# indianajohn/akaze-rust

Hardware: AMD Instinct MI355X
Metric: Mpix/s through extract_features (4 oct x 4 sub) (higher is better)
Workload: dtype f32

## Files before the change

akaze-rust_amd/csrc/akz_api.cpp:

```cpp
#include <cstdio>

#include "akz_ctx.hpp"

unsigned akz::host_cpu_share() {
    unsigned n = std::max(1u, std::thread::hardware_concurrency());
    cpu_set_t set;
    if (sched_getaffinity(0, sizeof(set), &set) == 0) n = std::max(1, CPU_COUNT(&set));
    if (FILE* f = fopen("/sys/fs/cgroup/cpu.max", "r")) {
        char q[32] = {0};
        long period = 0;
        if (fscanf(f, "%31s %ld", q, &period) == 2 && period > 0 && strcmp(q, "max") != 0)
            n = std::min<unsigned>(n, (unsigned)std::max(1L, atol(q) / period));
        fclose(f);
    }
    if (const char* e = std::getenv("LOCAL_WORLD_SIZE")) {
        const int ranks = atoi(e);
        if (ranks > 1) n = std::max(2u, n / (unsigned)ranks);
    }
    return std::max(1u, n);
}

int level_info_out(const std::vector<LevelPlan>& plan, uint64_t level, double* etime, double* esigma,
                          uint32_t* octave, uint32_t* sublevel, uint32_t* sigma_size, uint32_t* lw, uint32_t* lh,
                          uint32_t* det_sigma, uint64_t* n_tau, double* tau, uint64_t tau_cap) {
// ... 295 lines not shown
}
int akz_ctx_set_match_mode(akz_ctx* c, int mode) {
    AKZ_TRY(bind(c));
    if (mode < 0 || mode > 3) return AKZ_ERR_INVALID_ARG;
    c->settings.match_mode = mode;
    push_settings(c);
    return AKZ_OK;
}
int akz_ctx_set_fed_mode(akz_ctx* c, int mode) {
    AKZ_TRY(bind(c));
    if (mode != 0 && mode != 2) return AKZ_ERR_INVALID_ARG;
    c->settings.fed_mode = mode;
    push_settings(c);
    return AKZ_OK;
}
const char* akz_fed_kernel_name(void) { return "k_level_march + k_fed_own"; }
int akz_debug_march_bands(int kind, uint32_t w, uint32_t h, uint32_t n, int half_width, int32_t* rows, uint32_t cap,
                          uint32_t* n_bands) {
    if (!n_bands || (cap && !rows) || kind < 0 || kind > 1 || w < 16 || h < 16 || n == 0 || half_width < 1 || half_width > 4)
        return AKZ_ERR_INVALID_ARG;
    *n_bands = launch::march_band_rows(kind, w, h, n, half_width, rows, cap);
    return AKZ_OK;
}
int akz_debug_detector_set_cells(int half_width, const uint32_t* w, const uint32_t* h, uint32_t n_entries, uint32_t n, int32_t* cells,
                                 uint32_t cap, int32_t* grids, uint32_t* n_workgroups) {
    if (!n_workgroups || !w || !h || !grids || (cap && !cells) || n_entries < 1 || n_entries > launch::detector_march_set_max() || n == 0 ||
        half_width < 1 || half_width > 4)
        return AKZ_ERR_INVALID_ARG;
    for (uint32_t e = 0; e < n_entries; ++e)
        if (w[e] < 4u * (uint32_t)half_width + 8u || h[e] < 4u * (uint32_t)half_width + 8u) return AKZ_ERR_INVALID_ARG;
    *n_workgroups = launch::detector_set_cells(half_width, w, h, n_entries, n, cells, cap, grids);
    return AKZ_OK;
}
const char* akz_detector_kernel_name(void) { return "detector (k_detector_march + k_detector_tiled)"; }
int akz_debug_set_schedule(akz_ctx* c, int key, int value) {
    if (!c || key < 0 || key >= SCHED_COUNT_) return AKZ_ERR_INVALID_ARG;
    AKZ_TRY(bind(c));
    CtxSettings& s = c->settings;
    s.sched[key] = value;
    if (key == SCHED_DET_BAND_ROWS || key == SCHED_LEVEL_BAND_ROWS)
        launch::march_min_band_rows(s.sched[SCHED_DET_BAND_ROWS], s.sched[SCHED_LEVEL_BAND_ROWS]);
    if (key == SCHED_DET_SETS) launch::detector_set_waves(value >= 11 && value <= 14 ? value - 10 : 0);
    if (key == SCHED_JOB_KPX) {
        s.big_px_sync = value > 0 ? (uint64_t)value * 1000u : gates::kBigPxSync;
        s.big_px_async = value > 0 ? (uint64_t)value * 1000u : gates::kBigPxAsync;
        s.lane_px = value > 0 ? (uint64_t)value * 1000u : gates::kLanePx;
    }
    push_settings(c);
    return AKZ_OK;
}
int akz_debug_placement_verdict(float spin_pair_ms, float tiny_pair_ms, float tiny_alone_ms, float spin_ms) {
    return akz::placement_verdict(spin_pair_ms, tiny_pair_ms, tiny_alone_ms, spin_ms);
}
int akz_debug_stream_placement(akz_ctx* c, int* info) {
    if (!c || !info) return AKZ_ERR_INVALID_ARG;
    AKZ_TRY(bind(c));
    info[0] = c->placed ? 1 : 0;
    info[1] = c->pre_mode;
    info[2] = c->place_replaced;
    info[3] = c->place_collisions + c->lane_collisions;
    return AKZ_OK;
}
int akz_debug_select_info(akz_ctx* c, int* info) {
    if (!c || !info) return AKZ_ERR_INVALID_ARG;
    AKZ_TRY(bind(c));
    const akz_ctx* q = c->lanes.empty() ? c : c->lanes[0];
    info[0] = q->sel_last_mode.load();
    info[1] = (int)q->sel_last_rounds.load();
    info[2] = (int)q->sel_last_fallback.load();
    info[3] = (int)q->last_total_cands.load();
    for (int k = 0; k < 4; ++k) info[4 + k] = (int)q->sel_last_ticks[k].load();
    return AKZ_OK;
}
int akz_debug_set_select(akz_ctx* c, int mode) {
    if (!c) return AKZ_ERR_INVALID_ARG;
// ... 140 lines not shown
```

akaze-rust_amd/csrc/akz_internal.hpp:

```cpp
#pragma once
#include <hip/hip_runtime.h>

#include <cstdint>
#include <functional>
#include <string>
#include <vector>

#include "../../include/akaze_hip.h"
#include "../../include/akaze_hip_debug.h"

namespace akz {

void set_error(const std::string& msg);
unsigned host_cpu_share();

using TrialsOnDevice = std::function<int(const float*, const float*, const float*, const float*, uint32_t, const uint32_t*, uint32_t,
                                         float, float, float*, int32_t*)>;
int remove_outliers_impl(const akz_keypoint* keypoints_0, uint64_t n0, const akz_keypoint* keypoints_1, uint64_t n1,
                         const akz_match* matches, uint64_t n_matches, uint64_t num_trials, float epsilon_model,
                         float epsilon_inlier, akz_match* out, uint64_t* n_out, const TrialsOnDevice& trials_on_device);

#define AKZ_HIP_TRY(expr)                                                                          \
    do {                                                                                           \
        hipError_t _e = (expr);                                                                    \
// ... 156 lines not shown
    uint32_t w, h, level;
    float border_m;
};
uint32_t detector_tiled_set_max();
void detector_tiled_set(hipStream_t s, uint32_t sigma, const DetLevelDesc* levels, uint32_t nlevels, uint32_t n, float thr,
                        Candidate* d_cand, uint32_t cap, uint32_t* d_count);
void detector_tiled_fused(hipStream_t s, const float* lsmooth, uint32_t sigma, float* lx, float* ly, float* lxx,
                          float* lyy, float* lxy, float* ldet_out, uint32_t w, uint32_t h, uint32_t n, uint32_t level,
                          float thr, float border_m, Candidate* d_cand, uint32_t cap, uint32_t* d_count);
bool blur5_stream_supported(uint32_t w, uint32_t h, uint32_t ntaps, bool is_u8);
void blur5_stream_u8(hipStream_t s, const uint8_t* in, float* out, uint32_t w, uint32_t h, uint32_t n, const float* k);
void blur5_stream_f32(hipStream_t s, const float* in, float* out, uint32_t w, uint32_t h, uint32_t n, const float* k);
uint32_t march_band_rows(int kind, uint32_t w, uint32_t h, uint32_t n, int S, int32_t* cs_ce, uint32_t cap);
bool blur5_march_supported(uint32_t w, uint32_t h, uint32_t ntaps);
void blur5_march_u8(hipStream_t s, const uint8_t* in, float* out, uint32_t w, uint32_t h, uint32_t n, const float* k);
void blur5_march_f32(hipStream_t s, const float* in, float* out, uint32_t w, uint32_t h, uint32_t n, const float* k);
bool contrast_march_supported(uint32_t w, uint32_t h, uint32_t ntaps, uint32_t nbins);
void contrast_march(hipStream_t s, const float* in, uint32_t w, uint32_t h, uint32_t n, const float* g3,
                    unsigned long long* d_hmax_bits, uint32_t nbins, uint32_t* d_hist, double* d_thr);
void contrast_thresholds(hipStream_t s, const unsigned long long* d_hmax_bits, uint32_t nbins, uint32_t n, double* d_thr);
bool contrast_stream_supported(uint32_t w, uint32_t h, uint32_t ntaps, uint32_t nbins);
void contrast_stream(hipStream_t s, const float* in, uint32_t w, uint32_t h, uint32_t n, const float* g3,
                     unsigned long long* d_hmax_bits, uint32_t nbins, uint32_t* d_hist, double* d_thr);
bool prep_stream_supported(uint32_t w, uint32_t h);
void prep_stream(hipStream_t s, const float* prev, bool half, float* lt_out, float* lsmooth, float* lflow, uint32_t w,
                 uint32_t h, uint32_t pw, uint32_t ph, uint32_t n, const float* g3, const double* d_k, uint32_t k_pow);
bool detector_march_supported(uint32_t sigma, uint32_t w, uint32_t h, float border_m, bool nms);
void detector_march(hipStream_t s, const float* lsmooth, uint32_t sigma, float* lx, float* ly, float* lxx, float* lyy,
                    float* lxy, float* ldet_out, uint32_t w, uint32_t h, uint32_t n, uint32_t level, float thr,
                    float border_m, Candidate* d_cand, uint32_t cap, uint32_t* d_count);
uint32_t detector_march_set_max();
void detector_march_set(hipStream_t s, uint32_t sigma, const DetLevelDesc* levels, uint32_t nlevels, uint32_t n, float thr,
                        Candidate* d_cand, uint32_t cap, uint32_t* d_count);
void detector_set_waves(int waves);
uint32_t detector_set_cells(int S, const uint32_t* w, const uint32_t* h, uint32_t nlv, uint32_t n, int32_t* cells, uint32_t cap,
                            int32_t* grids);
bool head_fused_supported(uint32_t w, uint32_t h, uint32_t ntaps0, uint32_t ntaps1);
void head_fused_u8(hipStream_t s, const uint8_t* in, float* lt0, float* blurred, float* gx, float* gy, uint32_t w, uint32_t h, uint32_t n,
                   const float* k5, const float* g3, unsigned long long* d_smax_bits, uint32_t* d_zero_word = nullptr);
void head_fused_f32(hipStream_t s, const float* in, float* lt0, float* blurred, float* gx, float* gy, uint32_t w, uint32_t h, uint32_t n,
                    const float* k5, const float* g3, unsigned long long* d_smax_bits, uint32_t* d_zero_word = nullptr);
void contrast_hist_final(hipStream_t s, const float* gx, const float* gy, uint32_t w, uint32_t h, uint32_t n, unsigned long long* d_smax_bits,
                         uint32_t nbins, uint32_t* d_hist, uint32_t* d_done, double percentile, double* d_k);
void flow_from_pair(hipStream_t s, const float* gx, const float* gy, float* lflow, uint32_t w, uint32_t h, uint32_t n, const double* d_k,
                    uint32_t k_pow);
void march_min_band_rows(int detector, int level);
bool level_march_supported(uint32_t w, uint32_t h);
bool level_march_half_supported(uint32_t w, uint32_t h, uint32_t pw, uint32_t ph, uint32_t n_steps);
void level_march(hipStream_t s, const float* prev, float* lsmooth, float* lflow, float* lt_out, float* lstep, uint32_t w,
                 uint32_t h, uint32_t n, const float* g3, const double* d_k, uint32_t k_pow, const float* half_taus,
                 uint32_t n_steps, uint32_t pw = 0, uint32_t ph = 0);
struct ResidentLevel {
    float *lt, *lsmooth, *lflow, *lstep;
    uint32_t w, h;
    bool half;
    uint32_t n_tau;
    const float* half_tau;
    uint32_t k_pow;
};
constexpr int kResidentMaxLevels = 10;
constexpr int kResidentMaxSteps = 448;
bool octave_resident_supported(uint32_t w, uint32_t h);
void octave_resident(hipStream_t s, const float* prev, uint32_t pw, uint32_t ph, uint32_t n, const ResidentLevel* levels,
                     uint32_t n_levels, const float* g3, const double* d_k);
bool detector_nms_fused_supported(uint32_t sigma);
void detector_nms_fused(hipStream_t s, const float* lsmooth, uint32_t sigma, float* lx, float* ly, float* lxx,
                        float* lyy, float* lxy, float* ldet_out, uint32_t w, uint32_t h, uint32_t n, uint32_t level,
                        float thr, float border_m, Candidate* d_cand, uint32_t cap, uint32_t* d_count);
void rcp_f64_to_f32(hipStream_t s, const double* x, float* out, uint64_t n);
// ... 172 lines not shown
```

akaze-rust_amd/csrc/akz_march.hip:

```cpp
#include <hip/hip_runtime.h>

#include <algorithm>
#include <cstdlib>
#include <type_traits>

#include "akz_internal.hpp"
#include "akz_pm_g2.hpp"

namespace akz {
namespace {

typedef float f2 __attribute__((ext_vector_type(2)));
typedef float f2u __attribute__((ext_vector_type(2), aligned(4)));

constexpr int MT = 256;
constexpr int MW = 2 * MT;
constexpr int HALO = 16;
constexpr int USE = MW - 2 * HALO;
constexpr int PAD = 8;
constexpr int ROW = MW + 2 * PAD;
constexpr int CBUF = 32;
#ifndef AKZ_MARCH_PF
#define AKZ_MARCH_PF 3
#endif
// ... 11 lines not shown
    return (int)((blockIdx.x & 7u) * (gridDim.x >> 3) + (blockIdx.x >> 3));
#else
    return (int)blockIdx.x;
#endif
}
__host__ __device__ __forceinline__ void uniform_band_rows(const MarchGrid& g, int band, int S, int h, int* cs, int* ce) {
    *cs = S + band * g.band_rows;
    const int e = *cs + g.band_rows;
    *ce = e < h - S ? e : h - S;
}
__host__ __device__ __forceinline__ void level_band_rows(const MarchGrid& g, int band, int h, int* cs, int* ce) {
    *cs = 1 + (band == 0 ? 0 : g.edge_rows + (band - 1) * g.band_rows);
    const int e = *cs + (band == 0 ? g.edge_rows : g.band_rows);
    *ce = band == g.nbands - 1 ? h - 1 : (e < h - 1 ? e : h - 1);
}
struct MarchNms {
    unsigned level;
    float thr;
    int xlo, xhi, ylo, yhi;
    Candidate* cand;
    unsigned cap;
    unsigned* count;
};

constexpr int kDetSetMax = 4;
struct DetMarchEntry {
    const float* ls;
    float *lx, *ly, *ldet, *lxx, *lyy, *lxy;
    int w, h;
    MarchGrid g;
    unsigned level;
    int xlo, xhi, ylo, yhi;
    int first;
};
struct DetMarchSet {
    DetMarchEntry e[kDetSetMax];
};
#if defined(__HIP_DEVICE_COMPILE__)
#define AKZ_UNIFORM(x) __builtin_amdgcn_readfirstlane(x)
#else
#define AKZ_UNIFORM(x) (x)
#endif
__host__ __device__ __forceinline__ bool det_set_cell(const DetMarchSet& set, int wg, int nwg, DetMarchEntry* E, int* entry, int* img,
                                                      int* band, int* strip) {
#if AKZ_MARCH_XCD
    const int xcd = wg & 7, j = wg >> 3;
    (void)nwg;
#else
    const int xcd = wg / (nwg >> 3), j = wg - xcd * (nwg >> 3);
#endif
    DetMarchEntry X = set.e[0];
    int e = 0, jl = j;
    const int f1 = set.e[1].first, f2 = set.e[2].first, f3 = set.e[3].first;
    if (j >= f1) { X = set.e[1]; e = 1; jl = j - f1; }
    if (j >= f2) { X = set.e[2]; e = 2; jl = j - f2; }
    if (j >= f3) { X = set.e[3]; e = 3; jl = j - f3; }
    static_assert(kDetSetMax == 4, "compare chain");
    const int cell = AKZ_UNIFORM(xcd * ((X.g.total + 7) >> 3) + jl);
    if (cell >= X.g.total) return false;
    const int per = X.g.nbands * X.g.nstrips;
    const int i = AKZ_UNIFORM(cell / per);
    const int rem = cell - i * per;
    const int b = AKZ_UNIFORM(rem / X.g.nstrips);
    *E = X;
    *entry = e;
    *img = i;
    *band = b;
    *strip = rem - b * X.g.nstrips;
    return true;
}

__device__ __forceinline__ int clampi(int v, int lo, int hi) { return v < lo ? lo : (v > hi ? hi : v); }
__device__ __forceinline__ f2 tap_main(f2 a, f2 b, f2 c, float kn, float kwn) {
    const f2 z = {0.0f, 0.0f};
    return ((z + kn * a) + kwn * b) + kn * c;
}
__device__ __forceinline__ f2 tap_off(f2 a, f2 c) {
    const f2 z = {0.0f, 0.0f};
    return (z - a) + c;
}

__device__ __forceinline__ void cands_flush(Candidate* buf, unsigned& n, const MarchNms& nms, int lane) {
    if (n == 0) return;
    unsigned base = 0;
    if (lane == 0) base = atomicAdd(nms.count, n);
    base = (unsigned)__builtin_amdgcn_readfirstlane((int)base);
    const uint4* src = reinterpret_cast<const uint4*>(buf);
    uint4* dst = reinterpret_cast<uint4*>(nms.cand);
    for (unsigned e = (unsigned)lane; e < 2u * n; e += 64u)
        if (base + (e >> 1) < nms.cap) dst[2 * (size_t)base + e] = src[e];
    __builtin_amdgcn_wave_barrier();
    n = 0;
}
template <typename F>
__device__ __forceinline__ void cands_push(Candidate* buf, unsigned& n, unsigned m, const MarchNms& nms, int lane, F&& make) {
    while (__ballot(m != 0u)) {
        const bool have = m != 0u;
        const int i = have ? __ffs(m) - 1 : 0;
        m &= m - 1u;
        const unsigned long long b = __ballot(have);
        const unsigned nb = (unsigned)__popcll(b);
        if (n + nb > (unsigned)CBUF) cands_flush(buf, n, nms, lane);
        const unsigned before = (unsigned)__popcll(b & ((1ull << lane) - 1ull));
// ... 68 lines not shown
    constexpr int AUX = NT ? 2 : 0;
    if (!ODDW) {
        const unsigned vo = on ? C.vo_st : VO_NONE;
#pragma unroll
        for (int i = 0; i < N; ++i)
            __builtin_amdgcn_raw_buffer_store_b64(__builtin_bit_cast(u2, v[i]), plane[i], (int)vo, (int)ro, AUX);
    } else {
        const unsigned vo0 = on ? C.vo_st : VO_NONE, vo1 = on ? C.vo_st1 : VO_NONE;
#pragma unroll
        for (int i = 0; i < N; ++i) {
            const float a = v[i].x, b = v[i].y;
            __builtin_amdgcn_raw_buffer_store_b32(__float_as_uint(a), plane[i], (int)vo0, (int)ro, AUX);
            __builtin_amdgcn_raw_buffer_store_b32(__float_as_uint(b), plane[i], (int)vo1, (int)ro, AUX);
        }
    }
}
template <int S, int N, bool ODDW, bool NT = true>
__device__ __forceinline__ void store_filled(const __amdgpu_buffer_rsrc_t (&plane)[N], const Cols& C, int w, int h, int r, bool on,
                                             const f2 (&v)[N]) {
    store_rows<N, ODDW, NT>(plane, r, w, on, C, v);
    if (on && (r == S || r == h - 1 - S)) {
        if (r == S) {
#pragma nounroll
            for (int y = 0; y < S; ++y) store_rows<N, ODDW, NT>(plane, y, w, true, C, v);
        }
        if (r == h - 1 - S) {
#pragma nounroll
            for (int y = h - S; y < h; ++y) store_rows<N, ODDW, NT>(plane, y, w, true, C, v);
        }
    }
}

template <int S, bool NMS, bool KEEP, bool ODDW>
__global__ void __launch_bounds__(MT, 3)
k_detector_march(DetMarchSet set, float kn, float kwn, float quat, float thr, Candidate* __restrict__ cand, unsigned cap,
                 unsigned* __restrict__ count) {
    constexpr int P = 2 * S + 1, NOUT = KEEP ? 4 : 1;
    static_assert(2 * S + 2 <= HALO, "strip halo");
    constexpr int R = P % 3 == 0 ? 3 : P;
    constexpr int PF = AKZ_MARCH_PF < R - 1 ? AKZ_MARCH_PF : R - 1;
    static_assert(S <= PAD, "LDS padding");
    __shared__ __attribute__((aligned(16))) float s_row[2][4][ROW];
    __shared__ Candidate s_cands[NMS ? MT / 64 : 1][NMS ? CBUF : 1];
    const int tid = threadIdx.x, lane = tid & 63;
    const int wv = __builtin_amdgcn_readfirstlane(tid >> 6);
    Candidate* const cbuf = s_cands[NMS ? wv : 0];
    unsigned cnum = 0;
    DetMarchEntry E;
    int entry, img, band, strip;
    if (!det_set_cell(set, (int)blockIdx.x, (int)gridDim.x, &E, &entry, &img, &band, &strip)) return;
    const float* __restrict__ const ls = E.ls;
    float* __restrict__ const lx_out = E.lx;
    float* __restrict__ const ly_out = E.ly;
    float* __restrict__ const lxx_out = E.lxx;
    float* __restrict__ const lyy_out = E.lyy;
    float* __restrict__ const lxy_out = E.lxy;
    float* __restrict__ const ldet_out = E.ldet;
    const int w = E.w, h = E.h;
    const MarchGrid g = E.g;
    const MarchNms nms{E.level, thr, E.xlo, E.xhi, E.ylo, E.yhi, cand, cap, count};
    int cs, ce;
    uniform_band_rows(g, band, S, h, &cs, &ce);
    if (cs >= ce) return;

    const int X0 = strip * USE - HALO;
    const int p0 = (2 * tid + HALO) & (MW - 1);
    const bool inner = p0 >= HALO && p0 < MW - HALO;
    const Cols C = make_cols(X0 + p0, inner, w);
    const int i0 = PAD + clampi(clampi(C.x0, S, w - 1 - S) - X0, 0, MW - 1) - S;
    const int i1 = PAD + clampi(clampi(C.x0 + 1, S, w - 1 - S) - X0, 0, MW - 1) - S;
    const int wi = PAD + p0;
    unsigned xok = 0;
    if (NMS) {
        if (inner && C.x0 < w && C.x0 >= nms.xlo && C.x0 <= nms.xhi) xok |= 1u;
        if (inner && C.x0 + 1 < w && C.x0 + 1 >= nms.xlo && C.x0 + 1 <= nms.xhi) xok |= 2u;
    }

    const size_t base = (size_t)img * (size_t)w * (size_t)h;
    const __amdgpu_buffer_rsrc_t in = plane_rsrc(ls + base, w, h);
    const __amdgpu_buffer_rsrc_t out1[2] = {plane_rsrc(lx_out + base, w, h), plane_rsrc(ly_out + base, w, h)};
    __amdgpu_buffer_rsrc_t out2[NOUT];
    out2[0] = plane_rsrc(ldet_out + base, w, h);
    if (KEEP) {
        out2[1] = plane_rsrc(lxx_out + base, w, h);
        out2[2] = plane_rsrc(lyy_out + base, w, h);
        out2[3] = plane_rsrc(lxy_out + base, w, h);
    }
    const __amdgpu_buffer_rsrc_t(&out2c)[NOUT] = out2;

    const int v0 = cs - 1 - 2 * S;
    const int T = (ce - cs) + 4 * S + 3;
    auto feed = [&](int t) -> f2 {
        return load_pair<ODDW>(in, (unsigned)clampi(v0 + min(t, T - 1), S, h - 1 - S) * ((unsigned)w * 4u), C);
    };
    f2 q[R];
#pragma unroll
// ... 64 lines not shown
                    if (KEEP) { o[1] = lxx; o[2] = lyy; o[3] = lxy; }
                    const f2(&oc)[NOUT] = o;
                    store_filled<S, NOUT, ODDW>(out2c, C, w, h, c, c >= cs && c < ce, oc);
                }
                if (NMS) {
                    const int y = c - 1;
                    if (y >= cs && y < ce && y >= nms.ylo && y <= nms.yhi) {
                        const float* dr = buf + 3 * ROW + wi;
                        const float left = dr[-1], right = dr[2];
                        const bool h0 = (dm1.x > nms.thr) & (dm1.x > dm1.y) & (dm1.x > left) & (dm1.x > dm2.x) & (dm1.x > det.x);
                        const bool h1 = (dm1.y > nms.thr) & (dm1.y > right) & (dm1.y > dm1.x) & (dm1.y > dm2.y) & (dm1.y > det.y);
                        const unsigned m = ((h0 ? 1u : 0u) | (h1 ? 2u : 0u)) & xok;
                        cands_push(cbuf, cnum, m, nms, lane, [&](int i) {
                            Candidate cd;
                            cd.level = nms.level;
                            cd.idx = (unsigned)(y * w + C.x0 + i);
                            cd.v = i == 0 ? dm1.x : dm1.y;
                            cd.xp = i == 0 ? dm1.y : right;
                            cd.xm = i == 0 ? left : dm1.x;
                            cd.yp = i == 0 ? det.x : det.y;
                            cd.ym = i == 0 ? dm2.x : dm2.y;
                            cd.img = (unsigned)img;
                            return cd;
                        });
                    }
                    dm2 = dm1;
                    dm1 = det;
                }
                lx_c = lx_n;
                ly_c = ly_n;
            }
        }
    }
    if (NMS) cands_flush(cbuf, cnum, nms, lane);
}

struct LevelTaus {
    float half_tau[4];
};
__device__ __forceinline__ f2 lds2(const float* p) { return f2{p[0], p[1]}; }
__device__ __forceinline__ f2 tap3(f2 a, f2 b, f2 c, float k0, float k1, float k2) {
    const f2 z = {0.0f, 0.0f};
    return ((z + k0 * a) + k1 * b) + k2 * c;
}
__device__ __forceinline__ double octave_contrast(double k, unsigned pow) {
    for (unsigned i = 0; i < pow; ++i) k = k * 0.75;
    return k;
}

typedef unsigned u4m __attribute__((ext_vector_type(4)));
template <int N, bool KEEPSTEP, bool ODDW, bool HALF = false>
__global__ void __launch_bounds__(MT, 3)
k_level_march(const float* __restrict__ prev, float* __restrict__ lsmooth_out, float* __restrict__ lflow_out,
              float* __restrict__ lt_out, float* __restrict__ lstep_out, int w, int h, MarchGrid g, float g0, float g1,
              float g2, float kn, float kwn, const double* __restrict__ d_k, unsigned k_pow, LevelTaus ht, int pw = 0, int ph = 0) {
    static_assert(!(HALF && ODDW), "the 2x2 mean is folded in for even level widths only");
    static_assert(N >= 1 && N <= 4, "fused diffusion steps");
    static_assert(N + 3 <= HALO, "strip halo");
    constexpr int NPL = 3 + N;
#ifndef AKZ_LEVEL_PF
#define AKZ_LEVEL_PF 2
#endif
    constexpr int PF = AKZ_LEVEL_PF;
    static_assert(PF >= 1 && PF <= 3, "prefetch ring");
    __shared__ __attribute__((aligned(16))) float s_row[2][NPL][ROW];
    const int tid = threadIdx.x;
    const int per = g.nbands * g.nstrips;
// ... 540 lines not shown

namespace launch {

static void admissible_range(uint32_t dim, float border_m, int* lo, int* hi) {
    auto out_lo = [&](int v) { return (roundf((float)v - border_m) - 1.0f) < 0.0f; };
    auto out_hi = [&](int v) { return (roundf((float)v + border_m) + 1.0f) >= (float)dim; };
    int a = 1, b = (int)dim - 2;
    while (a <= b && out_lo(a)) ++a;
    while (b >= a && out_hi(b)) --b;
    *lo = a;
    *hi = b;
}

bool detector_march_supported(uint32_t sigma, uint32_t w, uint32_t h, float border_m, bool nms) {
    if (sigma < 1 || sigma > 4) return false;
    if (w < 4 * sigma + 8 || h < 4 * sigma + 8) return false;
    if ((uint64_t)w * h > (1ull << 28)) return false;
    return !nms || border_m >= (float)(sigma + 2);
}


#ifndef AKZ_DET_FILL
#define AKZ_DET_FILL 3
#endif
#ifndef AKZ_DET_MINROWS
#define AKZ_DET_MINROWS 40
#endif
static int det_min_band_rows(uint32_t w, uint32_t n) {
    if (g_det_min_rows > 0) return g_det_min_rows;
    return (uint64_t)n * ((w + USE - 1) / USE) <= 4 ? 24 : AKZ_DET_MINROWS;
}
constexpr int kDetSetWaves = 1;
static int g_det_set_waves = 0;
void detector_set_waves(int waves) { g_det_set_waves = waves >= 1 && waves <= 4 ? waves : 0; }

static void plan_march_set(const DetLevelDesc* lv, uint32_t nlv, uint32_t n, int S, MarchGrid* grids) {
    if (nlv == 1) {
        dim3 gr;
        grids[0] = plan_march(lv[0].w, lv[0].h, n, S, &gr, AKZ_DET_FILL, det_min_band_rows(lv[0].w, n));
        return;
    }
    uint64_t strip_rows = 0;
    for (uint32_t e = 0; e < nlv; ++e) strip_rows += (uint64_t)n * ((lv[e].w + USE - 1) / USE) * (lv[e].h - 2 * (uint32_t)S);
    const uint64_t target = (uint64_t)march_cus() * AKZ_DET_FILL * (uint64_t)(g_det_set_waves ? g_det_set_waves : kDetSetWaves);
    for (uint32_t e = 0; e < nlv; ++e) {
        MarchGrid g;
        g.nstrips = (int)((lv[e].w + USE - 1) / USE);
        const long rows = (long)lv[e].h - 2 * S;
        const long want = (long)((target * (uint64_t)rows + strip_rows - 1) / strip_rows);
        const long nb = std::max<long>(1, std::min<long>(want, std::max<long>(1, rows / det_min_band_rows(lv[e].w, n))));
        g.band_rows = (int)((rows + nb - 1) / nb);
        g.edge_rows = g.band_rows;
        g.nbands = (int)((rows + g.band_rows - 1) / g.band_rows);
        g.total = (int)((long)n * g.nstrips * g.nbands);
        grids[e] = g;
    }
}
static unsigned make_det_set(const DetLevelDesc* lv, uint32_t nlv, uint32_t n, int S, bool nms, DetMarchSet* set) {
    MarchGrid grids[kDetSetMax];
    plan_march_set(lv, nlv, n, S, grids);
    int first = 0;
    for (uint32_t e = 0; e < (uint32_t)kDetSetMax; ++e) {
        DetMarchEntry& E = set->e[e];
        if (e >= nlv) {
            E = DetMarchEntry{};
            E.first = 0x7fffffff;
            continue;
        }
        E = DetMarchEntry{lv[e].lsmooth, lv[e].lx, lv[e].ly, lv[e].ldet, lv[e].lxx, lv[e].lyy, lv[e].lxy, (int)lv[e].w, (int)lv[e].h,
                          grids[e], lv[e].level, 0, -1, 0, -1, first};
        if (nms) {
            admissible_range(lv[e].w, lv[e].border_m, &E.xlo, &E.xhi);
            admissible_range(lv[e].h, lv[e].border_m, &E.ylo, &E.yhi);
        }
        first += (grids[e].total + 7) / 8;
    }
    return (unsigned)first * 8u;
}

template <int S, bool NMS, bool KEEP>
static void launch_detector_march(hipStream_t s, const DetMarchSet& set, unsigned nwg, bool oddw, float kn, float kwn, float quat, float thr,
                                  Candidate* d_cand, uint32_t cap, uint32_t* d_count) {
    if (oddw)
        hipLaunchKernelGGL((k_detector_march<S, NMS, KEEP, true>), dim3(nwg), dim3(MT), 0, s, set, kn, kwn, quat, thr, d_cand, cap, d_count);
    else
        hipLaunchKernelGGL((k_detector_march<S, NMS, KEEP, false>), dim3(nwg), dim3(MT), 0, s, set, kn, kwn, quat, thr, d_cand, cap, d_count);
}
#define AKZ_MARCH(S)                                                                                               \
    case S: {                                                                                                      \
        const unsigned nwg = make_det_set(levels, nlevels, n, S, d_cand != nullptr, &set);                         \
        if (d_cand && keep) launch_detector_march<S, true, true>(s, set, nwg, oddw, kn, kwn, quat, thr, d_cand, cap, d_count);    \
        else if (d_cand) launch_detector_march<S, true, false>(s, set, nwg, oddw, kn, kwn, quat, thr, d_cand, cap, d_count);      \
        else if (keep) launch_detector_march<S, false, true>(s, set, nwg, oddw, kn, kwn, quat, thr, d_cand, cap, d_count);        \
        else launch_detector_march<S, false, false>(s, set, nwg, oddw, kn, kwn, quat, thr, d_cand, cap, d_count);                 \
    } break;

uint32_t detector_march_set_max() { return (uint32_t)kDetSetMax; }
void detector_march_set(hipStream_t s, uint32_t sigma, const DetLevelDesc* levels, uint32_t nlevels, uint32_t n, float thr,
                        Candidate* d_cand, uint32_t cap, uint32_t* d_count) {
    if (nlevels == 0 || nlevels > (uint32_t)kDetSetMax) return;
    const Taps m = taps_scharr_main(sigma);
    const float kn = m.wgt[0], kwn = m.wgt[1];
    const float quat = (float)(sigma * sigma * sigma * sigma);
    const bool keep = levels[0].lxx && levels[0].lyy && levels[0].lxy;
    const bool oddw = (levels[0].w & 1u) != 0;
    DetMarchSet set;
    switch (sigma) {
        AKZ_MARCH(1) AKZ_MARCH(2) AKZ_MARCH(3) AKZ_MARCH(4)
        default: break;
    }
}
#undef AKZ_MARCH
void detector_march(hipStream_t s, const float* lsmooth, uint32_t sigma, float* lx, float* ly, float* lxx, float* lyy,
                    float* lxy, float* ldet_out, uint32_t w, uint32_t h, uint32_t n, uint32_t level, float thr,
                    float border_m, Candidate* d_cand, uint32_t cap, uint32_t* d_count) {
    const DetLevelDesc one{lsmooth, lx, ly, lxx, lyy, lxy, ldet_out, w, h, level, border_m};
    detector_march_set(s, sigma, &one, 1, n, thr, d_cand, cap, d_count);
}
uint32_t detector_set_cells(int S, const uint32_t* w, const uint32_t* h, uint32_t nlv, uint32_t n, int32_t* cells, uint32_t cap,
                            int32_t* grids) {
    DetLevelDesc lv[kDetSetMax] = {};
    for (uint32_t e = 0; e < nlv; ++e) {
        lv[e].w = w[e];
        lv[e].h = h[e];
    }
    DetMarchSet set;
    const unsigned nwg = make_det_set(lv, nlv, n, S, false, &set);
    for (uint32_t e = 0; e < nlv; ++e) {
        grids[3 * e] = set.e[e].g.nstrips;
        grids[3 * e + 1] = set.e[e].g.nbands;
        grids[3 * e + 2] = set.e[e].g.band_rows;
    }
    for (unsigned i = 0; i < nwg && i < cap; ++i) {
        DetMarchEntry E;
        int entry = -1, img = -1, band = -1, strip = -1;
        if (!det_set_cell(set, (int)i, (int)nwg, &E, &entry, &img, &band, &strip)) entry = img = band = strip = -1;
        cells[4 * i] = entry;
        cells[4 * i + 1] = img;
        cells[4 * i + 2] = band;
        cells[4 * i + 3] = strip;
    }
    return nwg;
}

bool blur5_march_supported(uint32_t w, uint32_t h, uint32_t ntaps) {
    return ntaps == 5 && w >= 16 && h >= 16 && (uint64_t)w * h <= (1ull << 28);
}
template <typename T>
static void blur5_march_t(hipStream_t s, const T* in, float* out, uint32_t w, uint32_t h, uint32_t n, const float* k) {
    BlurTaps5 tp;
    for (int i = 0; i < 5; ++i) tp.k[i] = k[i];
    dim3 gr;
    const MarchGrid mg = plan_march(w, h, n, 2, &gr, 6, g_head_min_rows > 0 ? g_head_min_rows : 32);
    if (w & 1u) hipLaunchKernelGGL((k_blur5_march<T, true>), gr, dim3(MT), 0, s, in, out, (int)w, (int)h, mg, tp);
    else hipLaunchKernelGGL((k_blur5_march<T, false>), gr, dim3(MT), 0, s, in, out, (int)w, (int)h, mg, tp);
}
void blur5_march_u8(hipStream_t s, const uint8_t* in, float* out, uint32_t w, uint32_t h, uint32_t n, const float* k) {
    blur5_march_t<uint8_t>(s, in, out, w, h, n, k);
}
void blur5_march_f32(hipStream_t s, const float* in, float* out, uint32_t w, uint32_t h, uint32_t n, const float* k) {
    blur5_march_t<float>(s, in, out, w, h, n, k);
}

bool contrast_march_supported(uint32_t w, uint32_t h, uint32_t ntaps, uint32_t nbins) {
    return ntaps == 3 && nbins >= 1 && nbins <= 640 && level_march_supported(w, h);
}
void contrast_march(hipStream_t s, const float* in, uint32_t w, uint32_t h, uint32_t n, const float* g3,
                    unsigned long long* d_hmax_bits, uint32_t nbins, uint32_t* d_hist, double* d_thr) {
    const Taps m = taps_scharr_main(1);
    const ContrastMarchArgs ca{d_hmax_bits, d_hist, nbins, d_thr};
    dim3 gr;
    const MarchGrid mg = plan_level_march(w, h, n, &gr, 8, g_head_min_rows > 0 ? g_head_min_rows : 32);
    if (w & 1u)
        hipLaunchKernelGGL((k_contrast_march<1, true>), gr, dim3(MT), 0, s, in, (int)w, (int)h, mg, g3[0], g3[1], g3[2], m.wgt[0], m.wgt[1], ca);
    else
// ... 76 lines not shown
```

akaze-rust_amd/python/akaze_amd.py:

```python
import ctypes as C
import os

import numpy as np

_PKG = os.path.dirname(os.path.dirname(os.path.abspath(__file__)))
LIB_PATH = os.environ.get("AKAZE_HIP_LIB") or os.path.join(_PKG, "libakaze_hip.so")

AKZ_KEEP_ALL_PLANES = 1
AKZ_NO_HOST_DESCRIPTORS = 2
AKZ_NO_DETECT = 4
AKZ_INPUT_READY = 8
AKZ_ERR_BUFFER = -7

PLANES = ["Lt", "Lsmooth", "Lx", "Ly", "Lxx", "Lyy", "Lxy", "Lflow", "Lstep", "Ldet"]

FRAME_GRAY8, FRAME_RGB8, FRAME_BGR8, FRAME_RGBA8, FRAME_BGRA8, FRAME_RGB8_PLANAR = range(6)
KR_FRAME_LUMA = 12


class AkazeError(RuntimeError):
    def __init__(self, status, msg):
        super().__init__(f"akaze_hip status {status}: {msg}")
        self.status = status

# ... 236 lines not shown
        "akz_random_color": ([vp], i32),
        "akz_draw_circle": ([vp, u32, u32, C.c_float, C.c_float, vp, C.c_float], i32),
        "akz_draw_line": ([vp, u32, u32, C.c_float, C.c_float, C.c_float, C.c_float, vp, C.c_float], i32),
        "akz_job_abandon": ([vp], i32),
        "akz_result_free": ([vp], i32),
        "akz_result_num_images": ([vp, pu64], i32),
        "akz_result_counts": ([vp, u64, pu64, pu64, pu64], i32),
        "akz_result_keypoints": ([vp, u64, vp], i32),
        "akz_result_descriptors": ([vp, u64, vp], i32),
        "akz_result_device_descriptors": ([vp, u64, C.POINTER(vp), pu64], i32),
        "akz_result_contrast": ([vp, u64, pf64], i32),
        "akz_result_copy_device_descriptors": ([vp, vp, u64, pu64], i32),
        "akz_result_level_info": ([vp, u64, pf64, pf64, pu32, pu32, pu32, pu32, pu32, pu64, pf64, u64], i32),
        "akz_fetch_plane": ([vp, u64, u64, i32, vp, pu64], i32),
        "akz_fetch_pyramid": ([vp, u64, vp, u64, pu64], i32),
        "akz_result_device_plane": ([vp, u64, u64, i32, C.POINTER(vp)], i32),
        "akz_descriptor_match": ([vp, vp, u64, vp, u64, u64, u64, f64, vp, pu64], i32),
        "akz_descriptor_match_device": ([vp, vp, u64, vp, u64, u64, f64, vp, vp], i32),
        "akz_ctx_graph_probe": ([vp, vp, u32, u32, u32, C.POINTER(Config), u32, u32, pf64, pf64, pu64], i32),
        "akz_debug_march_bands": ([i32, u32, u32, u32, i32, C.POINTER(i32), u32, pu32], i32),
        "akz_ctx_set_lanes": ([vp, u32], i32),
        "akz_ctx_set_eager_finish": ([vp, i32], i32),
        "akz_fed_kernel_name": ([], C.c_char_p),
        "akz_ctx_set_host_threads": ([vp, u32], i32),
        "akz_debug_set_match_chunks": ([vp, u32, u32], i32),
        "akz_debug_set_host_sort": ([vp, i32], i32),
        "akz_debug_set_alloc_fill": ([vp, i32], i32),
        "akz_debug_audit_scratch": ([vp, vp, u32, pu32], i32),
        "akz_debug_resource_counts": ([pu64], i32),
        "akz_debug_set_select": ([vp, i32], i32),
        "akz_debug_select_info": ([vp, C.POINTER(C.c_int)], i32),
        "akz_debug_set_schedule": ([vp, i32, i32], i32),
        "akz_debug_detector_set_cells": ([i32, pu32, pu32, u32, u32, C.POINTER(i32), u32, C.POINTER(i32), pu32], i32),
        "akz_debug_stream_placement": ([vp, C.POINTER(i32)], i32),
        "akz_detector_kernel_name": ([], C.c_char_p),
        "akz_remove_outliers": ([vp, u64, vp, u64, vp, u64, u64, C.c_float, C.c_float, vp, pu64], i32),
        "akz_estimate_fundamental_matrix": ([vp, u64, vp, u64, vp, C.c_float, fp, C.POINTER(i32)], i32),
        "akz_match_features": ([vp, vp, u64, vp, u64, vp, u64, vp, u64, u64, f64, u64, C.c_float, vp, pu64], i32),
        "akz_match_features_pairs": ([vp, vp, u64, vp, u64, u64, f64, u64, C.c_float, vp, pu64], i32),
        "akz_debug_ransac_samples": ([u64, u64, u64, u64, pu64], i32),
        "akz_debug_ransac_samples_k": ([u64, u64, u64, u64, i32, pu64], i32),
        "akz_estimate_homography": ([vp, u64, vp, u64, vp, C.c_float, fp, C.POINTER(i32)], i32),
        "akz_remove_outliers_homography": ([vp, u64, vp, u64, vp, u64, u64, C.c_float, C.c_float, vp, pu64, fp, C.POINTER(i32)], i32),
        "akz_match_features_homography": ([vp, vp, u64, vp, u64, vp, u64, vp, u64, u64, f64, u64, C.c_float, vp, pu64, fp,
                                           C.POINTER(i32)], i32),
        "akz_match_features_homography_pairs": ([vp, vp, u64, vp, u64, u64, f64, u64, C.c_float, vp, pu64, fp, C.POINTER(i32)], i32),
        "akz_refine_homography": ([vp, u64, vp, u64, vp, u64, fp, C.c_float, C.c_uint32, vp, pu64, fp, C.POINTER(C.c_uint32)], i32),
        "akz_match_features_homography_refined": ([vp, vp, u64, vp, u64, vp, u64, vp, u64, u64, f64, u64, C.c_float, C.c_uint32, vp, pu64,
                                                   fp, C.POINTER(i32), C.POINTER(C.c_uint32)], i32),
        "akz_match_features_homography_refined_pairs": ([vp, vp, u64, vp, u64, u64, f64, u64, C.c_float, C.c_uint32, vp, pu64, fp,
                                                         C.POINTER(i32), C.POINTER(C.c_uint32)], i32),
        "akz_match_features_homography_refined_guided": ([vp, vp, u64, vp, u64, vp, u64, vp, u64, u64, f64, u64, C.c_float, C.c_uint32,
                                                          C.c_float, f64, vp, pu64, fp, C.POINTER(i32), C.POINTER(C.c_uint32)], i32),
        "akz_match_features_homography_refined_guided_pairs": ([vp, vp, u64, vp, u64, u64, f64, u64, C.c_float, C.c_uint32, C.c_float, f64,
                                                                vp, pu64, fp, C.POINTER(i32), C.POINTER(C.c_uint32)], i32),
        "akz_descriptor_match_guided_host": ([vp, u64, vp, u64, vp, u64, vp, u64, u64, i32, fp, C.c_float, u64, f64, vp, pu64], i32),
        "akz_descriptor_match_guided": ([vp, vp, u64, vp, u64, vp, u64, vp, u64, u64, i32, fp, C.c_float, u64, f64, vp, pu64], i32),
        "akz_descriptor_match_guided_pairs": ([vp, vp, u64, vp, u64, u64, i32, fp, C.c_float, u64, f64, vp, pu64], i32),
        "akz_match_features_homography_guided": ([vp, vp, u64, vp, u64, vp, u64, vp, u64, u64, f64, u64, C.c_float, C.c_float, f64, vp,
                                                  pu64, fp, C.POINTER(i32)], i32),
        "akz_match_features_homography_guided_pairs": ([vp, vp, u64, vp, u64, u64, f64, u64, C.c_float, C.c_float, f64, vp, pu64, fp,
                                                        C.POINTER(i32)], i32),
        "akz_remove_outliers_fundamental": ([vp, u64, vp, u64, vp, u64, u64, C.c_float, C.c_float, vp, pu64, fp, C.POINTER(i32)], i32),
        "akz_refine_fundamental_matrix": ([vp, u64, vp, u64, vp, u64, fp, C.c_float, C.c_uint32, vp, pu64, fp, C.POINTER(C.c_uint32)], i32),
        "akz_match_features_fundamental": ([vp, vp, u64, vp, u64, vp, u64, vp, u64, u64, f64, u64, C.c_float, vp, pu64, fp,
                                            C.POINTER(i32)], i32),
# ... 1899 lines not shown
```

include/akaze_hip_debug.h:

```cpp
#ifndef AKAZE_HIP_DEBUG_H
#define AKAZE_HIP_DEBUG_H
#include "akaze_hip.h"
#ifdef __cplusplus
extern "C" {
#endif

int akz_ctx_graph_probe(akz_ctx* ctx, const uint8_t* d_imgs, uint32_t w, uint32_t h, uint32_t n, const akz_config* cfg,
                        uint32_t flags, uint32_t reps, double* ms_graph, double* ms_plain, uint64_t* graph_nodes);
int akz_debug_march_bands(int kind, uint32_t w, uint32_t h, uint32_t n, int half_width, int32_t* rows, uint32_t cap,
                          uint32_t* n_bands);
int akz_debug_detector_set_cells(int half_width, const uint32_t* w, const uint32_t* h, uint32_t n_entries, uint32_t n, int32_t* cells,
                                 uint32_t cap, int32_t* grids, uint32_t* n_workgroups);
const char* akz_fed_kernel_name(void);
const char* akz_detector_kernel_name(void);
int akz_debug_set_match_chunks(akz_ctx* ctx, uint32_t pair_chunks, uint32_t set_chunks);
int akz_debug_match_tile_rows(uint32_t* rows);
int akz_debug_set_knn_chunks(akz_ctx* ctx, uint32_t chunks);
int akz_debug_set_schedule(akz_ctx* ctx, int key, int value);
int akz_debug_stream_placement(akz_ctx* ctx, int* info);
int akz_debug_placement_verdict(float spin_pair_ms, float tiny_pair_ms, float tiny_alone_ms, float spin_ms);
int akz_debug_device_libm(akz_ctx* ctx, int* available, int* last_job);
int akz_debug_set_device_libm(akz_ctx* ctx, int mode);
int akz_debug_libm_eval(akz_ctx* ctx, const float* d_a, const float* d_b, float* d_out3, uint64_t n, int fma);
typedef struct akz_gate {
    const char* name;
    double value;
    const char* unit;
    const char* meaning;
} akz_gate;
int akz_debug_gates(const akz_gate** rows, uint64_t* n);
int akz_ctx_calibrate_gates(akz_ctx* ctx, uint64_t* sync_px, uint64_t* async_px, double* ms);
enum { AKZ_KR_LEVEL_MARCH = 1, AKZ_KR_FED_OWN = 2, AKZ_KR_OCTAVE_RESIDENT = 3, AKZ_KR_DETECTOR_TILED = 4, AKZ_KR_DETECTOR_MARCH = 5,
       AKZ_KR_JPEG_IDCT = 6, AKZ_KR_JPEG_LUMA = 7, AKZ_KR_JPEG_COPY = 8, AKZ_KR_SORT_ROWS = 9, AKZ_KR_SORT_BUCKETS = 10,
       AKZ_KR_SORT_RADIX = 11, AKZ_KR_FRAME_LUMA = 12 };
typedef struct akz_kernel_row {
    uint32_t stage, kind, param, w, h, n;
    uint64_t launches, px, px_steps;
    double ms;
} akz_kernel_row;
int akz_debug_kernel_rows(akz_ctx* ctx, akz_kernel_row* out, uint32_t cap, uint32_t* n_rows, int reset);
int akz_debug_rcp_f64_to_f32(akz_ctx* ctx, const double* d_x, float* d_out, uint64_t n);
int akz_debug_set_host_sort(akz_ctx* ctx, int on);
int akz_debug_set_select(akz_ctx* ctx, int mode);
int akz_debug_select_info(akz_ctx* ctx, int* info);

// ... 27 lines not shown
```

Measured before the change: 15160.

## Schedule detector march as per-XCD row runs spanning levels and strips

The multi-level detector march kernel can now hand each workgroup a contiguous run of rows. A run is drawn from a per-XCD share of all set entries' (image, strip, row) units, so one workgroup can cover several strips or levels in sequence instead of one fixed band cell. The per-piece body is moved into a device helper, and the kernel loops over pieces with a barrier between them. The goal is to balance uneven level sizes across XCDs and CUs and cut tail imbalance and idle workgroups. The cost is extra index arithmetic and barriers per piece. The run plan falls back to the old cell grid when runs would be shorter than the minimum band rows. A debug API to enumerate pieces and a schedule knob to select the form are also added.

```diff
diff --git a/akaze-rust_amd/csrc/akz_api.cpp b/akaze-rust_amd/csrc/akz_api.cpp
--- a/akaze-rust_amd/csrc/akz_api.cpp
+++ b/akaze-rust_amd/csrc/akz_api.cpp
@@ -351,6 +351,16 @@
     *n_workgroups = launch::detector_set_cells(half_width, w, h, n_entries, n, cells, cap, grids);
     return AKZ_OK;
 }
+int akz_debug_detector_set_runs(int half_width, const uint32_t* w, const uint32_t* h, uint32_t n_entries, uint32_t n, int cell_rows, int waves,
+                                int32_t* pieces, uint32_t cap, uint32_t* n_pieces, uint32_t* n_workgroups) {
+    if (!n_workgroups || !n_pieces || !w || !h || (cap && !pieces) || n_entries < 1 || n_entries > launch::detector_march_set_max() || n == 0 ||
+        half_width < 1 || half_width > 4 || cell_rows < 0 || waves < 0 || waves > 4)
+        return AKZ_ERR_INVALID_ARG;
+    for (uint32_t e = 0; e < n_entries; ++e)
+        if (w[e] < 4u * (uint32_t)half_width + 8u || h[e] < 4u * (uint32_t)half_width + 8u) return AKZ_ERR_INVALID_ARG;
+    *n_workgroups = launch::detector_set_runs(half_width, w, h, n_entries, n, cell_rows, waves, pieces, cap, n_pieces);
+    return *n_workgroups ? AKZ_OK : AKZ_ERR_INVALID_ARG;
+}
 const char* akz_detector_kernel_name(void) { return "detector (k_detector_march + k_detector_tiled)"; }
 int akz_debug_set_schedule(akz_ctx* c, int key, int value) {
     if (!c || key < 0 || key >= SCHED_COUNT_) return AKZ_ERR_INVALID_ARG;
@@ -359,7 +369,7 @@
     s.sched[key] = value;
     if (key == SCHED_DET_BAND_ROWS || key == SCHED_LEVEL_BAND_ROWS)
         launch::march_min_band_rows(s.sched[SCHED_DET_BAND_ROWS], s.sched[SCHED_LEVEL_BAND_ROWS]);
-    if (key == SCHED_DET_SETS) launch::detector_set_waves(value >= 11 && value <= 14 ? value - 10 : 0);
+    if (key == SCHED_DET_SETS) launch::detector_set_sched(value);
     if (key == SCHED_JOB_KPX) {
         s.big_px_sync = value > 0 ? (uint64_t)value * 1000u : gates::kBigPxSync;
         s.big_px_async = value > 0 ? (uint64_t)value * 1000u : gates::kBigPxAsync;
diff --git a/akaze-rust_amd/csrc/akz_internal.hpp b/akaze-rust_amd/csrc/akz_internal.hpp
--- a/akaze-rust_amd/csrc/akz_internal.hpp
+++ b/akaze-rust_amd/csrc/akz_internal.hpp
@@ -212,9 +212,11 @@
 uint32_t detector_march_set_max();
 void detector_march_set(hipStream_t s, uint32_t sigma, const DetLevelDesc* levels, uint32_t nlevels, uint32_t n, float thr,
                         Candidate* d_cand, uint32_t cap, uint32_t* d_count);
-void detector_set_waves(int waves);
+void detector_set_sched(int value);
 uint32_t detector_set_cells(int S, const uint32_t* w, const uint32_t* h, uint32_t nlv, uint32_t n, int32_t* cells, uint32_t cap,
                             int32_t* grids);
+uint32_t detector_set_runs(int S, const uint32_t* w, const uint32_t* h, uint32_t nlv, uint32_t n, int cell_rows, int waves, int32_t* pieces,
+                           uint32_t cap, uint32_t* n_pieces);
 bool head_fused_supported(uint32_t w, uint32_t h, uint32_t ntaps0, uint32_t ntaps1);
 void head_fused_u8(hipStream_t s, const uint8_t* in, float* lt0, float* blurred, float* gx, float* gy, uint32_t w, uint32_t h, uint32_t n,
                    const float* k5, const float* g3, unsigned long long* d_smax_bits, uint32_t* d_zero_word = nullptr);
diff --git a/akaze-rust_amd/csrc/akz_march.hip b/akaze-rust_amd/csrc/akz_march.hip
--- a/akaze-rust_amd/csrc/akz_march.hip
+++ b/akaze-rust_amd/csrc/akz_march.hip
@@ -67,9 +67,12 @@
     unsigned level;
     int xlo, xhi, ylo, yhi;
     int first;
+    unsigned units;
 };
 struct DetMarchSet {
     DetMarchEntry e[kDetSetMax];
+    int runs;
+    unsigned run_rows;
 };
 #if defined(__HIP_DEVICE_COMPILE__)
 #define AKZ_UNIFORM(x) __builtin_amdgcn_readfirstlane(x)
@@ -104,6 +107,68 @@
     *strip = rem - b * X.g.nstrips;
     return true;
 }
+struct DetRun {
+    unsigned xcd, pos, end;
+};
+__host__ __device__ __forceinline__ DetMarchEntry det_set_entry(const DetMarchSet& set, int e) {
+#if defined(__HIP_DEVICE_COMPILE__)
+    (void)set;
+    const DetMarchSet* const args = (const DetMarchSet*)__builtin_amdgcn_kernarg_segment_ptr();
+    return args->e[e];
+#else
+    return set.e[e];
+#endif
+}
+__host__ __device__ __forceinline__ unsigned det_run_share(unsigned units, unsigned xcd) { return (units * xcd) >> 3; }
+__host__ __device__ __forceinline__ unsigned det_run_sequence(const DetMarchSet& set, unsigned xcd) {
+    unsigned u = 0;
+#pragma unroll
+    for (int e = 0; e < kDetSetMax; ++e) u += det_run_share(set.e[e].units, xcd + 1) - det_run_share(set.e[e].units, xcd);
+    return u;
+}
+__host__ __device__ __forceinline__ bool det_run_cell(const DetMarchSet& set, int wg, int nwg, DetRun* R) {
+#if AKZ_MARCH_XCD
+    const unsigned xcd = (unsigned)wg & 7u, j = (unsigned)wg >> 3;
+    (void)nwg;
+#else
+    const unsigned xcd = (unsigned)(wg / (nwg >> 3)), j = (unsigned)wg - xcd * (unsigned)(nwg >> 3);
+#endif
+    const unsigned len = det_run_sequence(set, xcd);
+    const unsigned pos = j * set.run_rows;
+    R->xcd = xcd;
+    R->pos = pos;
+    R->end = pos + set.run_rows < len ? pos + set.run_rows : len;
+    return pos < len;
+}
+__host__ __device__ __forceinline__ void det_run_piece(const DetMarchSet& set, int S, DetRun* R, DetMarchEntry* E, int* entry, int* img,
+                                                       int* strip, int* cs, int* ce) {
+    const unsigned x = R->xcd, p = R->pos;
+    const unsigned lo0 = det_run_share(set.e[0].units, x), lo1 = det_run_share(set.e[1].units, x);
+    const unsigned lo2 = det_run_share(set.e[2].units, x), lo3 = det_run_share(set.e[3].units, x);
+    const unsigned s1 = det_run_share(set.e[0].units, x + 1) - lo0, s2 = s1 + det_run_share(set.e[1].units, x + 1) - lo1;
+    const unsigned s3 = s2 + det_run_share(set.e[2].units, x + 1) - lo2, s4 = s3 + det_run_share(set.e[3].units, x + 1) - lo3;
+    static_assert(kDetSetMax == 4, "compare chain");
+    int e = 0;
+    unsigned at = lo0 + p, left = s1 - p;
+    if (p >= s1) { e = 1; at = lo1 + (p - s1); left = s2 - p; }
+    if (p >= s2) { e = 2; at = lo2 + (p - s2); left = s3 - p; }
+    if (p >= s3) { e = 3; at = lo3 + (p - s3); left = s4 - p; }
+    const DetMarchEntry X = det_set_entry(set, AKZ_UNIFORM(e));
+    const unsigned rows = (unsigned)(X.h - 2 * S);
+    const unsigned col = (unsigned)AKZ_UNIFORM((int)(at / rows));
+    const unsigned r = at - col * rows;
+    unsigned len = rows - r;
+    if (len > left) len = left;
+    if (len > R->end - p) len = R->end - p;
+    const unsigned i = (unsigned)AKZ_UNIFORM((int)(col / (unsigned)X.g.nstrips));
+    *E = X;
+    *entry = e;
+    *img = (int)i;
+    *strip = (int)(col - i * (unsigned)X.g.nstrips);
+    *cs = S + (int)r;
+    *ce = S + (int)(r + len);
+    R->pos = p + len;
+}
 
 __device__ __forceinline__ int clampi(int v, int lo, int hi) { return v < lo ? lo : (v > hi ? hi : v); }
 __device__ __forceinline__ f2 tap_main(f2 a, f2 b, f2 c, float kn, float kwn) {
@@ -238,23 +303,15 @@
 }
 
 template <int S, bool NMS, bool KEEP, bool ODDW>
-__global__ void __launch_bounds__(MT, 3)
-k_detector_march(DetMarchSet set, float kn, float kwn, float quat, float thr, Candidate* __restrict__ cand, unsigned cap,
-                 unsigned* __restrict__ count) {
+__device__ __forceinline__ void detector_piece(const DetMarchEntry& E, int img, int strip, int cs, int ce, float kn, float kwn, float quat,
+                                               float thr, Candidate* __restrict__ cand, unsigned cap, unsigned* __restrict__ count,
+                                               float (&s_row)[2][4][ROW], Candidate* cbuf, unsigned& cnum) {
     constexpr int P = 2 * S + 1, NOUT = KEEP ? 4 : 1;
     static_assert(2 * S + 2 <= HALO, "strip halo");
     constexpr int R = P % 3 == 0 ? 3 : P;
     constexpr int PF = AKZ_MARCH_PF < R - 1 ? AKZ_MARCH_PF : R - 1;
     static_assert(S <= PAD, "LDS padding");
-    __shared__ __attribute__((aligned(16))) float s_row[2][4][ROW];
-    __shared__ Candidate s_cands[NMS ? MT / 64 : 1][NMS ? CBUF : 1];
     const int tid = threadIdx.x, lane = tid & 63;
-    const int wv = __builtin_amdgcn_readfirstlane(tid >> 6);
-    Candidate* const cbuf = s_cands[NMS ? wv : 0];
-    unsigned cnum = 0;
-    DetMarchEntry E;
-    int entry, img, band, strip;
-    if (!det_set_cell(set, (int)blockIdx.x, (int)gridDim.x, &E, &entry, &img, &band, &strip)) return;
     const float* __restrict__ const ls = E.ls;
     float* __restrict__ const lx_out = E.lx;
     float* __restrict__ const ly_out = E.ly;
@@ -263,11 +320,7 @@
     float* __restrict__ const lxy_out = E.lxy;
     float* __restrict__ const ldet_out = E.ldet;
     const int w = E.w, h = E.h;
-    const MarchGrid g = E.g;
     const MarchNms nms{E.level, thr, E.xlo, E.xhi, E.ylo, E.yhi, cand, cap, count};
-    int cs, ce;
-    uniform_band_rows(g, band, S, h, &cs, &ce);
-    if (cs >= ce) return;
 
     const int X0 = strip * USE - HALO;
     const int p0 = (2 * tid + HALO) & (MW - 1);
@@ -398,7 +451,40 @@
             }
         }
     }
-    if (NMS) cands_flush(cbuf, cnum, nms, lane);
+}
+
+template <int S, bool NMS, bool KEEP, bool ODDW>
+__global__ void __launch_bounds__(MT, 3)
+k_detector_march(DetMarchSet set, float kn, float kwn, float quat, float thr, Candidate* __restrict__ cand, unsigned cap,
+                 unsigned* __restrict__ count) {
+    __shared__ __attribute__((aligned(16))) float s_row[2][4][ROW];
+    __shared__ Candidate s_cands[NMS ? MT / 64 : 1][NMS ? CBUF : 1];
+    const int wv = __builtin_amdgcn_readfirstlane((int)threadIdx.x >> 6);
+    Candidate* const cbuf = s_cands[NMS ? wv : 0];
+    unsigned cnum = 0;
+    DetMarchEntry E;
+    int entry, img, band, strip;
+    int cs, ce;
+    const bool runs = set.runs != 0;
+    DetRun run{0u, 0u, 0u};
+    if (runs) {
+        if (!det_run_cell(set, (int)blockIdx.x, (int)gridDim.x, &run)) return;
+    } else {
+        if (!det_set_cell(set, (int)blockIdx.x, (int)gridDim.x, &E, &entry, &img, &band, &strip)) return;
+        uniform_band_rows(E.g, band, S, E.h, &cs, &ce);
+        if (cs >= ce) return;
+    }
+    for (bool first = true;; first = false) {
+        if (runs) {
+            if (run.pos >= run.end) break;
+            if (!first) __syncthreads();
+            det_run_piece(set, S, &run, &E, &entry, &img, &strip, &cs, &ce);
+        } else if (!first) {
+            break;
+        }
+        detector_piece<S, NMS, KEEP, ODDW>(E, img, strip, cs, ce, kn, kwn, quat, thr, cand, cap, count, s_row, cbuf, cnum);
+    }
+    if (NMS) cands_flush(cbuf, cnum, MarchNms{0u, thr, 0, -1, 0, -1, cand, cap, count}, (int)threadIdx.x & 63);
 }
 
 struct LevelTaus {
@@ -1005,7 +1091,11 @@
 }
 constexpr int kDetSetWaves = 1;
 static int g_det_set_waves = 0;
-void detector_set_waves(int waves) { g_det_set_waves = waves >= 1 && waves <= 4 ? waves : 0; }
+static int g_det_set_form = 0;
+void detector_set_sched(int value) {
+    g_det_set_waves = value >= 11 && value <= 14 ? value - 10 : (value >= 21 && value <= 24 ? value - 20 : 0);
+    g_det_set_form = value == 3 ? 3 : (value == 0 || (value >= 21 && value <= 24) ? 0 : 2);
+}
 
 static void plan_march_set(const DetLevelDesc* lv, uint32_t nlv, uint32_t n, int S, MarchGrid* grids) {
     if (nlv == 1) {
@@ -1029,9 +1119,30 @@
         grids[e] = g;
     }
 }
-static unsigned make_det_set(const DetLevelDesc* lv, uint32_t nlv, uint32_t n, int S, bool nms, DetMarchSet* set) {
+static unsigned plan_det_runs(DetMarchSet* set, uint32_t w0, uint32_t n, int form, int cell_rows, int waves) {
+    if (form == 2) return 0;
+    unsigned longest = 0, total = 0;
+    for (int e = 0; e < kDetSetMax; ++e) total += set->e[e].units;
+    if (total >= (1u << 28)) return 0;
+    for (unsigned x = 0; x < 8; ++x) longest = std::max(longest, det_run_sequence(*set, x));
+    if (longest == 0) return 0;
+    const unsigned per_xcd = std::max(1u, (unsigned)(march_cus() * AKZ_DET_FILL * (waves ? waves : kDetSetWaves)) / 8u);
+    unsigned L = (longest + per_xcd - 1) / per_xcd;
+    if (form == 3) {
+        if (cell_rows > 0) L = std::min((unsigned)cell_rows, longest);
+    } else if (L < (unsigned)det_min_band_rows(w0, n)) {
+        return 0;
+    }
+    set->runs = 1;
+    set->run_rows = L;
+    return (longest + L - 1) / L * 8u;
+}
+static unsigned make_det_set(const DetLevelDesc* lv, uint32_t nlv, uint32_t n, int S, bool nms, DetMarchSet* set, int form, int cell_rows,
+                             int waves) {
     MarchGrid grids[kDetSetMax];
     plan_march_set(lv, nlv, n, S, grids);
+    set->runs = 0;
+    set->run_rows = 0;
     int first = 0;
     for (uint32_t e = 0; e < (uint32_t)kDetSetMax; ++e) {
         DetMarchEntry& E = set->e[e];
@@ -1041,13 +1152,16 @@
             continue;
         }
         E = DetMarchEntry{lv[e].lsmooth, lv[e].lx, lv[e].ly, lv[e].ldet, lv[e].lxx, lv[e].lyy, lv[e].lxy, (int)lv[e].w, (int)lv[e].h,
-                          grids[e], lv[e].level, 0, -1, 0, -1, first};
+                          grids[e], lv[e].level, 0, -1, 0, -1, first, 0u};
+        const uint64_t units = (uint64_t)n * (uint64_t)grids[e].nstrips * (lv[e].h - 2 * (uint32_t)S);
+        E.units = (unsigned)std::min<uint64_t>(units, 1u << 28);
         if (nms) {
             admissible_range(lv[e].w, lv[e].border_m, &E.xlo, &E.xhi);
             admissible_range(lv[e].h, lv[e].border_m, &E.ylo, &E.yhi);
         }
         first += (grids[e].total + 7) / 8;
     }
+    if (const unsigned nwg = plan_det_runs(set, lv[0].w, n, form, cell_rows, waves)) return nwg;
     return (unsigned)first * 8u;
 }
 
@@ -1061,7 +1175,8 @@
 }
 #define AKZ_MARCH(S)                                                                                               \
     case S: {                                                                                                      \
-        const unsigned nwg = make_det_set(levels, nlevels, n, S, d_cand != nullptr, &set);                         \
+        const unsigned nwg = make_det_set(levels, nlevels, n, S, d_cand != nullptr, &set, g_det_set_form,         \
+                                          g_det_min_rows, g_det_set_waves);                                       \
         if (d_cand && keep) launch_detector_march<S, true, true>(s, set, nwg, oddw, kn, kwn, quat, thr, d_cand, cap, d_count);    \
         else if (d_cand) launch_detector_march<S, true, false>(s, set, nwg, oddw, kn, kwn, quat, thr, d_cand, cap, d_count);      \
         else if (keep) launch_detector_march<S, false, true>(s, set, nwg, oddw, kn, kwn, quat, thr, d_cand, cap, d_count);        \
@@ -1098,7 +1213,7 @@
         lv[e].h = h[e];
     }
     DetMarchSet set;
-    const unsigned nwg = make_det_set(lv, nlv, n, S, false, &set);
+    const unsigned nwg = make_det_set(lv, nlv, n, S, false, &set, 2, 0, g_det_set_waves);
     for (uint32_t e = 0; e < nlv; ++e) {
         grids[3 * e] = set.e[e].g.nstrips;
         grids[3 * e + 1] = set.e[e].g.nbands;
@@ -1114,6 +1229,31 @@
         cells[4 * i + 3] = strip;
     }
     return nwg;
+}
+uint32_t detector_set_runs(int S, const uint32_t* w, const uint32_t* h, uint32_t nlv, uint32_t n, int cell_rows, int waves, int32_t* pieces,
+                           uint32_t cap, uint32_t* n_pieces) {
+    DetLevelDesc lv[kDetSetMax] = {};
+    for (uint32_t e = 0; e < nlv; ++e) {
+        lv[e].w = w[e];
+        lv[e].h = h[e];
+    }
+    DetMarchSet set;
+    const unsigned nwg = make_det_set(lv, nlv, n, S, false, &set, 3, cell_rows, waves);
+    uint32_t k = 0;
+    for (unsigned i = 0; set.runs && i < nwg; ++i) {
+        DetRun run;
+        if (!det_run_cell(set, (int)i, (int)nwg, &run)) continue;
+        for (; run.pos < run.end; ++k) {
+            DetMarchEntry E;
+            int entry, img, strip, cs, ce;
+            det_run_piece(set, S, &run, &E, &entry, &img, &strip, &cs, &ce);
+            if (k >= cap) continue;
+            const int32_t rec[6] = {(int32_t)i, entry, img, strip, cs, ce - cs};
+            std::copy(rec, rec + 6, pieces + 6 * (size_t)k);
+        }
+    }
+    *n_pieces = k;
+    return set.runs ? nwg : 0;
 }
 
 bool blur5_march_supported(uint32_t w, uint32_t h, uint32_t ntaps) {
diff --git a/akaze-rust_amd/python/akaze_amd.py b/akaze-rust_amd/python/akaze_amd.py
--- a/akaze-rust_amd/python/akaze_amd.py
+++ b/akaze-rust_amd/python/akaze_amd.py
@@ -292,6 +292,7 @@
         "akz_debug_select_info": ([vp, C.POINTER(C.c_int)], i32),
         "akz_debug_set_schedule": ([vp, i32, i32], i32),
         "akz_debug_detector_set_cells": ([i32, pu32, pu32, u32, u32, C.POINTER(i32), u32, C.POINTER(i32), pu32], i32),
+        "akz_debug_detector_set_runs": ([i32, pu32, pu32, u32, u32, i32, i32, C.POINTER(i32), u32, pu32, pu32], i32),
         "akz_debug_stream_placement": ([vp, C.POINTER(i32)], i32),
         "akz_detector_kernel_name": ([], C.c_char_p),
         "akz_remove_outliers": ([vp, u64, vp, u64, vp, u64, u64, C.c_float, C.c_float, vp, pu64], i32),
diff --git a/include/akaze_hip_debug.h b/include/akaze_hip_debug.h
--- a/include/akaze_hip_debug.h
+++ b/include/akaze_hip_debug.h
@@ -11,6 +11,8 @@
                           uint32_t* n_bands);
 int akz_debug_detector_set_cells(int half_width, const uint32_t* w, const uint32_t* h, uint32_t n_entries, uint32_t n, int32_t* cells,
                                  uint32_t cap, int32_t* grids, uint32_t* n_workgroups);
+int akz_debug_detector_set_runs(int half_width, const uint32_t* w, const uint32_t* h, uint32_t n_entries, uint32_t n, int cell_rows,
+                                int waves, int32_t* pieces, uint32_t cap, uint32_t* n_pieces, uint32_t* n_workgroups);
 const char* akz_fed_kernel_name(void);
 const char* akz_detector_kernel_name(void);
 int akz_debug_set_match_chunks(akz_ctx* ctx, uint32_t pair_chunks, uint32_t set_chunks);
```

Result: no change. 15220 (median of 6 runs) (+0.4%).
